# leavesnight/VIEO_SLAM

Hardware: AMD Instinct MI355X
Metric: frontend+localBA frames/sec on EuRoC MH05 stereo-VIO; ATE vs ref (higher is better)
Workload: dtype u8 (extract/match) + f64 (pose optimisation)

## Files before the change

### vieo_slam_amd/csrc/orb_extractor.hip

```cpp
#include <algorithm>
#include <cmath>
#include <type_traits>
#include <vector>

#include "../../include/vieo_orb_pattern_31.h"
#include "common.h"
#include "sincosf_exact.h"
#include "wave_ops.h"

#define QT_DEVICE
#include "quadtree.inl"

#include "orb_internal.h"

namespace vieo {

#ifndef VIEO_RESIZE_ROWS
#define VIEO_RESIZE_ROWS 32
#endif
static const int kResizeRows = VIEO_RESIZE_ROWS;
#ifndef VIEO_QT_GROUPS
#define VIEO_QT_GROUPS {1, 64}
#endif

// ... 156 lines not shown
    const short4 y = yt2[dy];
    const uint8_t* r0 = l1 + (y.x - ry0) * kL1P;
    const uint8_t* r1 = l1 + (y.y - ry0) * kL1P;
    const int b0 = y.z, b1 = y.w;
    unsigned out = 0;
#pragma unroll
    for (int j = 0; j < 4; j++) {
      const int h0 = r0[x0[j]] * a0[j] + r0[x1[j]] * a1[j];
      const int h1 = r1[x0[j]] * a0[j] + r1[x1[j]] * a1[j];
      const int v = (((b0 * (int)(unsigned short)(h0 >> 4)) >> 16) + ((b1 * (int)(unsigned short)(h1 >> 4)) >> 16) + 2) >> 2;
      out |= (unsigned)(v & 0xFF) << (8 * j);
    }
    *(unsigned*)(dst2 + (size_t)dy * D2.pitch + dx4) = out & keep;
  }
}

#ifndef VIEO_XCD_RUN
#define VIEO_XCD_RUN 32
#endif
static const int kXcdRun = VIEO_XCD_RUN;
__device__ __forceinline__ int xcd_grouped(int bid, int G) {
  const int xcd = bid & 7, q = bid >> 3;
  return ((q / G) * 8 + xcd) * G + q % G;
}

__device__ __forceinline__ int min3i(int a, int b, int c) { return min(min(a, b), c); }
__device__ __forceinline__ int max3i(int a, int b, int c) { return max(max(a, b), c); }

__device__ __forceinline__ int fast_strength(const uint8_t* t, int p) {
  const int v = t[0];
  int d[16];
  d[0] = v - t[3 * p];
  d[1] = v - t[3 * p + 1];
  d[2] = v - t[2 * p + 2];
  d[3] = v - t[p + 3];
  d[4] = v - t[3];
  d[5] = v - t[-p + 3];
  d[6] = v - t[-2 * p + 2];
  d[7] = v - t[-3 * p + 1];
  d[8] = v - t[-3 * p];
  d[9] = v - t[-3 * p - 1];
  d[10] = v - t[-2 * p - 2];
  d[11] = v - t[-p - 3];
  d[12] = v - t[-3];
  d[13] = v - t[p - 3];
  d[14] = v - t[2 * p - 2];
  d[15] = v - t[3 * p - 1];
  int lo3[16], hi3[16];
#pragma unroll
  for (int k = 0; k < 16; k++) {
    lo3[k] = min3i(d[k], d[(k + 1) & 15], d[(k + 2) & 15]);
    hi3[k] = max3i(d[k], d[(k + 1) & 15], d[(k + 2) & 15]);
  }
  int A = -256, B = 256;
#pragma unroll
  for (int k = 0; k < 16; k++) {
    A = max(A, min3i(lo3[k], lo3[(k + 3) & 15], lo3[(k + 6) & 15]));
    B = min(B, max3i(hi3[k], hi3[(k + 3) & 15], hi3[(k + 6) & 15]));
  }
  return max(max(A, -B), 0);
}

#ifdef VIEO_FAST_STATS
__device__ unsigned long long g_fast_stats[8];
#define FAST_STAT(i, v) do { if (lane == 0) atomicAdd(&g_fast_stats[i], (unsigned long long)(v)); } while (0)
#else
#define FAST_STAT(i, v) do { } while (0)
#endif

__device__ __forceinline__ bool fast_compass(const uint8_t* t, int p, int th) {
  const int v = t[0], lo = v - th, hi = v + th;
  const int x0 = t[3 * p], x4 = t[3], x8 = t[-3 * p], x12 = t[-3];
  const bool dk = ((x0 < lo) | (x8 < lo)) & ((x4 < lo) | (x12 < lo));
  const bool br = ((x0 > hi) | (x8 > hi)) & ((x4 > hi) | (x12 > hi));
  return dk | br;
}

__device__ __forceinline__ void wave_sync() {
  __builtin_amdgcn_fence(__ATOMIC_RELEASE, "wavefront");
  __builtin_amdgcn_wave_barrier();
  __builtin_amdgcn_fence(__ATOMIC_ACQUIRE, "wavefront");
}

__device__ __forceinline__ void fast_cell(const OrbParams& P, const CellDesc& cd, int b, int c, uint8_t* tile, uint8_t* sc,
                                          unsigned short* cand, int cand_cap, int tpitch, int iniTh, int minTh, int lane,
                                          unsigned* __restrict__ cell_keys, int* __restrict__ cell_counts) {
  const int x0a = cd.x0 & ~3;
  const int vw = cd.cw - 6, vh = cd.ch - 6;
  const int npx = (vw > 0 && vh > 0) ? vw * vh : 0;
  const int sp = vw + 2;
  if (npx > 0)
    for (int idx = lane; idx < ((vh + 2) * sp + 15) / 16; idx += 64) ((uint4*)sc)[idx] = make_uint4(0, 0, 0, 0);
  wave_sync();
  const int xo = cd.x0 - x0a;
  unsigned* out = cell_keys + ((size_t)b * P.ncells + c) * P.cell_cap;
  int base = 0;
  for (int round = 0; round < 2 && base == 0; round++) {
    if (round == 1 && minTh >= iniTh) break;
    const int th = round == 0 ? iniTh : minTh;
    int na = 0, nc = 0;
    bool overflow = false;
    FAST_STAT(round, 1);
    auto pass_b = [&]() {
      int w = nc;
      FAST_STAT(3, (na - nc + 63) / 64);
      FAST_STAT(6, na - nc);
      for (int i0 = nc; i0 < na; i0 += 64) {
        const int i = i0 + lane;
        bool pass = false;
        int p = 0;
        if (i < na) {
          p = cand[i];
          const int y = p >> 6, x = p & 63;
          const int r = fast_strength(tile + (y + 3) * tpitch + (x + 3 + xo), tpitch);
          sc[(y + 1) * sp + x + 1] = (uint8_t)r;
          pass = r > th;
        }
        const unsigned long long m = __ballot(pass);
        if (pass) cand[w + __popcll(m & ((1ull << lane) - 1ull))] = (unsigned short)p;
        w += __popcll(m);
      }
      nc = na = w;
    };
    if (npx > 0) {
      const int s = __builtin_amdgcn_readfirstlane((3 + xo) & 3), kq = (3 + xo) >> 2;
      const int ng = (vw + 3) >> 2, G = ng * vh;
      const int qy = 64 / ng, rx = 64 - qy * ng;
      const unsigned H = 0x80808080u, T = (unsigned)th * 0x01010101u;
      const unsigned Tl = T & ~H;
      auto ltu = [&](unsigned a, unsigned bb) -> unsigned {
        const unsigned d = (a | H) - (bb & ~H);
        return __builtin_amdgcn_bitop3_b32(a, bb, d, 0x4D);
      };
      auto pass_a = [&](auto SC) {
        constexpr int S = decltype(SC)::value;
        int y = lane / ng, lx4 = lane - y * ng;
        int toff = y * tpitch + 4 * lx4;
        const int step_off = qy * tpitch + 4 * rx, wrap_off = tpitch - 4 * ng;
        const uint8_t* base_u = tile + 4 * kq;
        const uint8_t* base_c = base_u + 3 * tpitch;
        const uint8_t* base_d = base_u + 6 * tpitch;
        const unsigned Htail = (unsigned)(0x80808080ull & ((1ull << (8 * (vw - 4 * (ng - 1)))) - 1ull));
        for (int g0 = 0; g0 < G; g0 += 64) {
          if (na + 256 > cand_cap) {
            wave_sync();
            pass_b();
            wave_sync();
            if (na + 256 > cand_cap) {
              overflow = true;
              break;
            }
          }
          unsigned m4 = 0;
          const int x0 = 4 * lx4;
          if (g0 + lane < G) {
            const unsigned* rc = (const unsigned*)(base_c + toff);
            const unsigned* ru = (const unsigned*)(base_u + toff);
            const unsigned* rd = (const unsigned*)(base_d + toff);
            unsigned C, L, R, U, D;
            if constexpr (S == 0) {
              const unsigned wm = rc[-1], w0 = rc[0], w1 = rc[1];
              C = w0, U = ru[0], D = rd[0], L = __builtin_amdgcn_alignbyte(w0, wm, 1), R = __builtin_amdgcn_alignbyte(w1, w0, 3);
            } else if constexpr (S == 1) {
              const unsigned wm = rc[-1], w0 = rc[0], w1 = rc[1];
              C = __builtin_amdgcn_alignbyte(w1, w0, 1), U = __builtin_amdgcn_alignbyte(ru[1], ru[0], 1),
              D = __builtin_amdgcn_alignbyte(rd[1], rd[0], 1), L = __builtin_amdgcn_alignbyte(w0, wm, 2), R = w1;
            } else if constexpr (S == 2) {
              const unsigned wm = rc[-1], w0 = rc[0], w1 = rc[1], w2 = rc[2];
              C = __builtin_amdgcn_alignbyte(w1, w0, 2), U = __builtin_amdgcn_alignbyte(ru[1], ru[0], 2),
              D = __builtin_amdgcn_alignbyte(rd[1], rd[0], 2), L = __builtin_amdgcn_alignbyte(w0, wm, 3),
              R = __builtin_amdgcn_alignbyte(w2, w1, 1);
            } else {
              const unsigned w0 = rc[0], w1 = rc[1], w2 = rc[2];
              C = __builtin_amdgcn_alignbyte(w1, w0, 3), U = __builtin_amdgcn_alignbyte(ru[1], ru[0], 3),
              D = __builtin_amdgcn_alignbyte(rd[1], rd[0], 3), L = w0, R = __builtin_amdgcn_alignbyte(w2, w1, 2);
            }
            const unsigned ge = ~ltu(C, T) & H;
            const unsigned gem = (ge - (ge >> 7)) | ge;
            const unsigned dif = ((C | H) - Tl) ^ ((C ^ ~T) & H);
            const unsigned lo = dif & gem;
            const unsigned suml = (C & ~H) + Tl;
            const unsigned sum = suml ^ ((C ^ T) & H);
            const unsigned cy = __builtin_amdgcn_bitop3_b32(C, T, suml, 0xE8) & H;
            const unsigned hi = sum | ((cy - (cy >> 7)) | cy);
            const unsigned dk = (ltu(U, lo) | ltu(D, lo)) & (ltu(L, lo) | ltu(R, lo));
            const unsigned br = (ltu(hi, U) | ltu(hi, D)) & (ltu(hi, L) | ltu(hi, R));
            const unsigned f = (dk | br) & (lx4 == ng - 1 ? Htail : H);
            m4 = ((f >> 7) * 0x01020408u) >> 24;
          }
          const int cnt = __popc(m4);
          int inc = cnt;
          inc += __builtin_amdgcn_update_dpp(0, inc, 0x111, 0xF, 0xF, true);
          inc += __builtin_amdgcn_update_dpp(0, inc, 0x112, 0xF, 0xF, true);
          inc += __builtin_amdgcn_update_dpp(0, inc, 0x114, 0xF, 0xF, true);
          inc += __builtin_amdgcn_update_dpp(0, inc, 0x118, 0xF, 0xF, true);
          inc += VIEO_DPP(0, inc, VIEO_DPP_ROW_BCAST15, 0xA);
          inc += VIEO_DPP(0, inc, VIEO_DPP_ROW_BCAST31, 0xC);
          int pos = na + inc - cnt;
          const unsigned key = (unsigned)((y << 6) | x0);
#pragma unroll
          for (int j = 0; j < 4; j++)
            if (m4 & (1u << j)) cand[pos++] = (unsigned short)(key + j);
          na += __builtin_amdgcn_readlane(inc, 63);
          lx4 += rx, y += qy, toff += step_off;
          if (lx4 >= ng) lx4 -= ng, y++, toff += wrap_off;
        }
      };
      if (s == 0) pass_a(std::integral_constant<int, 0>());
      else if (s == 1) pass_a(std::integral_constant<int, 1>());
      else if (s == 2) pass_a(std::integral_constant<int, 2>());
      else pass_a(std::integral_constant<int, 3>());
    }
    wave_sync();
    if (!overflow) pass_b();
    else {
      FAST_STAT(2, 1);
      for (int i0 = 0; i0 < npx; i0 += 64) {
        const int i = i0 + lane;
        if (i < npx) {
          const int y = i / vw, x = i - y * vw;
          sc[(y + 1) * sp + x + 1] = (uint8_t)fast_strength(tile + (y + 3) * tpitch + (x + 3 + xo), tpitch);
        }
      }
    }
    wave_sync();
    const int nC = overflow ? npx : nc;
    FAST_STAT(4, (nC + 63) / 64);
    for (int i0 = 0; i0 < nC; i0 += 64) {
      const int i = i0 + lane;
      bool keep = false;
      unsigned key = 0;
      if (i < nC) {
        int x, y;
        if (overflow) {
          y = i / vw, x = i - y * vw;
        } else {
          const int p = cand[i];
          y = p >> 6, x = p & 63;
        }
        const uint8_t* s = sc + (y + 1) * sp + x + 1;
        const int r = s[0];
        if (r > th) {
          const int sv = r - 1;
#define NB(o) ((s[o] > th) ? (int)s[o] - 1 : 0)
          keep = sv > NB(1) && sv > NB(-1) && sv > NB(-sp - 1) && sv > NB(-sp) && sv > NB(-sp + 1) &&
                 sv > NB(sp - 1) && sv > NB(sp) && sv > NB(sp + 1);
#undef NB
          key = (unsigned)(x + 3 + cd.offx) | ((unsigned)(y + 3 + cd.offy) << 12) |
                ((unsigned)sv << 24);
        }
      }
      const unsigned long long m = __ballot(keep);
      if (keep) {
        const int pos = base + __popcll(m & ((1ull << lane) - 1ull));
        if (pos < P.cell_cap) out[pos] = key;
      }
      base += __popcll(m);
    }
    wave_sync();
  }
  FAST_STAT(7, base);
  if (lane == 0) cell_counts[(size_t)b * P.ncells + c] = min(base, P.cell_cap);
}

#ifndef VIEO_FAST_WAVES
#define VIEO_FAST_WAVES 1
#endif
__global__ void __launch_bounds__(64 * VIEO_FAST_WAVES)
k_fast(OrbParams P, ImgSet I, const CellDesc* __restrict__ cells, unsigned* __restrict__ cell_keys,
       int* __restrict__ cell_counts, int iniTh, int minTh, int tpitch, int tile_bytes,
       int score_bytes, int cand_cap, int n_images, int lds_per_wave) {
  extern __shared__ __attribute__((aligned(16))) uint8_t smem_all[];
  const int lane = threadIdx.x & 63;
  const int wave_in_wg = __builtin_amdgcn_readfirstlane((int)(threadIdx.x >> 6));
  uint8_t* smem = smem_all + wave_in_wg * lds_per_wave;
  const int item = xcd_grouped(blockIdx.x, kXcdRun) * VIEO_FAST_WAVES + wave_in_wg;
  if (item >= P.ncells * n_images) return;
  const int b = item / P.ncells, c = item - b * P.ncells;
  const CellDesc cd = cells[c];
  int pitch;
  const uint8_t* src = plane_ptr(P, I, b, cd.level, &pitch);
  uint8_t* tile = smem;
  uint8_t* sc = smem + tile_bytes;
  unsigned short* cand = (unsigned short*)(smem + tile_bytes + score_bytes);
  const int x0a = cd.x0 & ~3;
  const int ndw = ((cd.x0 + cd.cw + 3) >> 2) - (x0a >> 2);
  {
    const int dc = lane & 15, dr = lane >> 4;
    const uint8_t* gbase = src + (size_t)cd.y0 * pitch + x0a;
    const unsigned gstep = 4u * (unsigned)pitch, tstep = 4u * (unsigned)tpitch;
    unsigned goff = (unsigned)dr * (unsigned)pitch + 4u * dc;
    uint8_t* t = tile + dr * tpitch + 4 * dc;
    const int kfull = cd.ch >> 2;
    if (dc < ndw) {
      unsigned v[16];
#pragma unroll
      for (int k = 0; k < 16; k++) {
        if (k < kfull)
          v[k] = *(const unsigned*)(gbase + goff);
        else if (dr + 4 * k < cd.ch)
          v[k] = *(const unsigned*)(gbase + goff);
        goff += gstep;
      }
#pragma unroll
      for (int k = 0; k < 16; k++) {
        if (k < kfull)
          *(unsigned*)t = v[k];
        else if (dr + 4 * k < cd.ch)
          *(unsigned*)t = v[k];
        t += tstep;
      }
      for (int r = dr + 64; r < cd.ch; r += 4, goff += gstep, t += tstep) *(unsigned*)t = *(const unsigned*)(gbase + goff);
    }
    for (int idx = lane; idx < cd.ch * (ndw - 16); idx += 64) {
      const int r = idx / (ndw - 16), dcol = 16 + idx % (ndw - 16);
      *(unsigned*)(tile + r * tpitch + 4 * dcol) =
          *(const unsigned*)(src + (size_t)(cd.y0 + r) * pitch + x0a + 4 * dcol);
    }
  }
  fast_cell(P, cd, b, c, tile, sc, cand, cand_cap, tpitch, iniTh, minTh, lane, cell_keys, cell_counts);
}

__global__ void __launch_bounds__(1024)
k_quadtree(OrbParams P, const unsigned* __restrict__ cell_keys,
           const int* __restrict__ cell_counts, unsigned* __restrict__ keys,
           unsigned short* __restrict__ kslot, unsigned char* __restrict__ kq,
           unsigned* __restrict__ sel, int* __restrict__ sel_count, int ncap_max, int scap_max, int l0) {
  extern __shared__ __attribute__((aligned(16))) uint8_t smem[];
  const int l = l0 + blockIdx.x, b = blockIdx.y;
  const LevelDesc& D = P.lv[l];
  uint8_t* q = smem;
  QtMem m;
  m.scanA = (unsigned long long*)q;
  q += sizeof(unsigned long long) * scap_max;
  m.scanB = (unsigned long long*)q;
  q += sizeof(unsigned long long) * scap_max;
  m.cnt = (int*)q;
  q += 4 * ncap_max;
  m.cc = (int*)q;
  q += 16 * ncap_max;
  m.best = (unsigned*)q;
  q += 4 * ncap_max;
  m.cand_size[0] = (int*)q;
  q += 4 * ncap_max;
  m.cand_size[1] = (int*)q;
  q += 4 * ncap_max;
  m.s = (QtShared*)q;
  q += 64;
  m.x0 = (short*)q;
  q += 2 * ncap_max;
  m.y0 = (short*)q;
  q += 2 * ncap_max;
  m.x1 = (short*)q;
  q += 2 * ncap_max;
  m.y1 = (short*)q;
  q += 2 * ncap_max;
  m.child = (unsigned short*)q;
  q += 8 * ncap_max;
  m.mark = (unsigned short*)q;
  q += 2 * ncap_max;
  m.list[0] = (unsigned short*)q;
  q += 2 * ncap_max;
  m.list[1] = (unsigned short*)q;
  q += 2 * ncap_max;
  m.cand_slot[0] = (unsigned short*)q;
  q += 2 * ncap_max;
  m.cand_slot[1] = (unsigned short*)q;
  q += 2 * ncap_max;
  m.order = (unsigned short*)q;
  q += 2 * ncap_max;
  m.flag = (unsigned char*)q;
  m.ncap = D.ncap;
  m.scap = scap_max;

  const int tid = threadIdx.x;
  const int ncell = D.cell_end - D.cell_begin;
  const int* cnts = cell_counts + (size_t)b * P.ncells + D.cell_begin;
  for (int i = tid; i < ncell; i += blockDim.x) m.scanA[i] = (unsigned long long)cnts[i];
  for (int i = tid; i < D.nIni; i += blockDim.x) m.cnt[i] = 0;
  __syncthreads();
  unsigned long long* inc = qt_scan(m.scanA, m.scanB, ncell);
  if (tid == 0) m.s->K = ncell > 0 ? (int)inc[ncell - 1] : 0;
  __syncthreads();
  const int K = m.s->K;
  unsigned* kk = keys + (size_t)b * P.keys_per_image + D.key_off;
  unsigned short* ks = kslot + (size_t)b * P.keys_per_image + D.key_off;
  unsigned char* kqq = kq + (size_t)b * P.keys_per_image + D.key_off;
  {
    const unsigned* cells0 = cell_keys + ((size_t)b * P.ncells + D.cell_begin) * P.cell_cap;
    const int nth = blockDim.x;
    for (int t0 = tid; t0 < K; t0 += 4 * nth) {
      unsigned key[4];
#pragma unroll
      for (int u = 0; u < 4; u++) {
        const int t = t0 + u * nth;
        key[u] = 0;
        if (t < K) {
          int lo = 0, hi = ncell - 1;
          while (lo < hi) {
            const int mid = (lo + hi) >> 1;
            if ((int)inc[mid] > t)
              hi = mid;
            else
// ... 706 lines not shown
    if (l > 0) {
      std::vector<short> t;
      D.xtab_off = (int)(xtab.size() / 4);
      resize_axis_table(P.lv[l - 1].w, D.w, true, t);
      xtab.insert(xtab.end(), t.begin(), t.end());
      D.ytab_off = (int)(ytab.size() / 4);
      resize_axis_table(P.lv[l - 1].h, D.h, false, t);
      ytab.insert(ytab.end(), t.begin(), t.end());
      const short* xt = xtab.data() + 4 * (size_t)D.xtab_off;
      const short* yt = ytab.data() + 4 * (size_t)D.ytab_off;
      for (int y0 = 0; y0 < D.h; y0 += kResizeRows)
        resize_rows = std::max(resize_rows, yt[4 * (std::min(y0 + kResizeRows, D.h) - 1) + 1] - yt[4 * y0] + 1);
      for (int x0 = 0; x0 < D.w; x0 += 256)
        resize_dw = std::max(resize_dw, ((xt[4 * (std::min(x0 + 256, D.w) - 1) + 1] + 4) >> 2) - (xt[4 * x0] >> 2));
    }
    D.tile_begin = (int)e->tiles.size();
    D.tiles_x = (D.w + kBlurTW - 1) / kBlurTW;
    for (int ty = 0; ty < (D.h + kBlurTH - 1) / kBlurTH; ty++)
      for (int tx = 0; tx < D.tiles_x; tx++) e->tiles.push_back({(short)l, (short)tx, (short)ty, 0});
    D.tile_end = (int)e->tiles.size();
  }
  P.ncells = (int)e->cells.size();
  if (max_cw - 6 > 64 || max_ch - 6 > 1023) {
    set_error("FAST cell wider than 64 pixels (image narrower than one 30-pixel cell?)");
    return VIEO_E_INVALID;
  }
  P.cell_cap = std::max(16, ((max_cw - 6 + 1) / 2) * ((max_ch - 6 + 1) / 2));
  for (int l = 0; l < e->nlevels; l++) {
    LevelDesc& D = P.lv[l];
    D.key_off = key_off;
    D.key_cap = (D.cell_end - D.cell_begin) * P.cell_cap;
    key_off += D.key_cap;
    if (D.key_cap >= (1 << 24)) {
      set_error("too many candidate keys per level");
      return VIEO_E_INVALID;
    }
  }
  P.keys_per_image = key_off;
  P.sel_per_image = sel_off;
  P.kp_cap = sel_off;
  e->ncap_max = ncap_max;
  e->scap_max = std::max(2 * ncap_max, max_ncell);
  e->pyr_img = align_up_sz(pyr_off, 256);
  e->blur_img = align_up_sz(blur_off, 256);
  e->resize_pitch = 4 * resize_dw + 4;
  e->resize_lds = resize_rows * e->resize_pitch;
  {
    bool ok = e->nlevels >= 3;
    int rows2 = 1, dw2 = 1;
    for (int l = 1; ok && l + 1 < e->nlevels; l += 2) {
      const LevelDesc &D1 = P.lv[l], &D2 = P.lv[l + 1];
      const short* xt1 = xtab.data() + 4 * (size_t)D1.xtab_off;
      const short* yt1 = ytab.data() + 4 * (size_t)D1.ytab_off;
      const short* xt2 = xtab.data() + 4 * (size_t)D2.xtab_off;
      const short* yt2 = ytab.data() + 4 * (size_t)D2.ytab_off;
      for (int ex0 = 0; ok && ex0 < D2.w; ex0 += kR2W) {
        const int ex1 = std::min(ex0 + kR2W, D2.w);
        const int rx0 = ex0 == 0 ? 0 : (xt2[4 * ex0] & ~3), rx1 = ex1 == D2.w ? D1.w : std::min(xt2[4 * (ex1 - 1) + 1] + 1, D1.w);
        const int ox1 = ex1 == D2.w ? D1.w : (xt2[4 * ex1] & ~3);
        const int ndw = ((xt1[4 * (rx1 - 1) + 1] + 4) >> 2) - ((xt1[4 * rx0] & ~3) >> 2);
        ok = rx1 - rx0 <= 256 && ox1 <= rx1 && ox1 > rx0 && ndw <= 128;
        dw2 = std::max(dw2, ndw);
      }
      for (int ey0 = 0; ok && ey0 < D2.h; ey0 += kR2H) {
        const int ey1 = std::min(ey0 + kR2H, D2.h);
        const int ry0 = ey0 == 0 ? 0 : yt2[4 * ey0], ry1 = ey1 == D2.h ? D1.h : std::min(yt2[4 * (ey1 - 1) + 1] + 1, D1.h);
        const int oy1 = ey1 == D2.h ? D1.h : yt2[4 * ey1];
        const int nrows = yt1[4 * (ry1 - 1) + 1] - yt1[4 * ry0] + 1;
        ok = ry1 - ry0 <= kR2Rows && oy1 <= ry1 && oy1 > ry0 && nrows <= 48;
        rows2 = std::max(rows2, nrows);
      }
    }
    e->resize2_ok = ok;
    e->resize2_pitch = 4 * dw2 + 4;
    e->resize2_l1_off = (rows2 * e->resize2_pitch + 15) & ~15;
    e->resize2_lds = e->resize2_l1_off + kR2Rows * 260;
  }
  e->tpitch = align_up(max_cw + 3, 4) + 4;
  e->tile_bytes = align_up(e->tpitch * max_ch, 16);
  e->score_bytes = align_up((max_cw - 4) * (max_ch - 4), 16) + 16;
  e->fast_cand_cap = std::max(256, std::min((max_cw - 6) * (max_ch - 6), 512));
  if (const char* cc = getenv("VIEO_FAST_CAND_CAP")) e->fast_cand_cap = std::max(256, atoi(cc));
  e->fast_lds = e->tile_bytes + e->score_bytes + align_up(2 * e->fast_cand_cap, 16) + 16;
  e->qt_lds = 16 * e->scap_max + (4 + 16 + 4 + 4 + 4) * ncap_max + 64 + (2 * 4 + 8 + 2 * 6) * ncap_max +
              ncap_max + 64;
  int rc;
#define ENS(buf, bytes)                 \
  if ((rc = (buf).ensure(bytes)) != VIEO_OK) return rc
  ENS(e->d_pyr, e->pyr_img * B);
  if (!orb_fused()) ENS(e->d_blur, e->blur_img * B);
  ENS(e->d_cells, e->cells.size() * sizeof(CellDesc));
  ENS(e->d_tiles, e->tiles.size() * sizeof(BlurTile));
  ENS(e->d_xtab, std::max<size_t>(xtab.size() * 2, 8));
  ENS(e->d_ytab, std::max<size_t>(ytab.size() * 2, 8));
  ENS(e->d_cell_keys, (size_t)B * P.ncells * P.cell_cap * 4);
  ENS(e->d_cell_counts, (size_t)B * P.ncells * 4);
  ENS(e->d_keys, (size_t)B * P.keys_per_image * 4);
  ENS(e->d_kslot, (size_t)B * P.keys_per_image * 2);
  ENS(e->d_kq, (size_t)B * P.keys_per_image);
  ENS(e->d_sel, (size_t)B * P.sel_per_image * 4);
  ENS(e->d_sel_count, (size_t)B * kMaxLevels * 4);
  ENS(e->d_tmp_kp, (size_t)B * P.kp_cap * sizeof(vieo_keypoint));
  ENS(e->d_tmp_desc, (size_t)B * P.kp_cap * 32);
  ENS(e->d_tmp_counts, (size_t)B * 2 * 4);
  ENS(e->d_krec, (size_t)B * P.kp_cap * 8);
#undef ENS
  VIEO_HIP_CHECK(hipMemcpyAsync(e->d_cells.p, e->cells.data(), e->cells.size() * sizeof(CellDesc),
                                hipMemcpyHostToDevice, e->stream));
  VIEO_HIP_CHECK(hipMemcpyAsync(e->d_tiles.p, e->tiles.data(), e->tiles.size() * sizeof(BlurTile),
                                hipMemcpyHostToDevice, e->stream));
  if (!xtab.empty()) {
    VIEO_HIP_CHECK(hipMemcpyAsync(e->d_xtab.p, xtab.data(), xtab.size() * 2, hipMemcpyHostToDevice,
                                  e->stream));
    VIEO_HIP_CHECK(hipMemcpyAsync(e->d_ytab.p, ytab.data(), ytab.size() * 2, hipMemcpyHostToDevice,
                                  e->stream));
  }
  VIEO_HIP_CHECK(hipStreamSynchronize(e->stream));
  if (e->qt_lds > 64 * 1024)
    VIEO_HIP_CHECK(hipFuncSetAttribute((const void*)k_quadtree,
                                       hipFuncAttributeMaxDynamicSharedMemorySize, e->qt_lds));
  if (e->qt_lds > 160 * 1024) {
    set_error("nfeatures too large for the LDS quadtree (%d bytes)", e->qt_lds);
    return VIEO_E_INVALID;
  }
  e->w = w;
  e->h = h;
  e->B = B;
  return VIEO_OK;
}

static int run_batch(vieo_orb* e, const uint8_t* d_images, int B, int w, int h, int stride,
                     size_t image_pitch, const int* lapping, vieo_keypoint* d_kp, uint8_t* d_desc,
                     int capacity, int32_t* d_counts) {
  int rc;
  if (w != e->w || h != e->h || B > e->B) {
    if ((rc = plan_geometry(e, w, h, std::max(B, (w == e->w && h == e->h) ? e->B : 0))) != VIEO_OK)
      return rc;
  }
  if ((stride & 3) || ((uintptr_t)d_images & 3) || (image_pitch & 3)) {
    set_error("device images need 4-byte aligned base, stride and pitch");
    return VIEO_E_INVALID;
  }
  const OrbParams& P = e->P;
  ImgSet I;
  I.img0 = d_images;
  I.stride0 = stride;
  I.img_pitch = image_pitch;
  I.pyr = e->d_pyr.as<uint8_t>();
  I.pyr_img = e->pyr_img;
  I.blur = e->d_blur.as<uint8_t>();
  I.blur_img = e->blur_img;
  e->last_imgs = I;
  e->last_B = B;
  hipStream_t st = e->stream;
  Timing& T = e->tm;
  int evi = 0;
  hipEvent_t* evs = T.ev[T.steps % kTimingRing];
#define STAMP()                                                  \
  if (T.on) VIEO_HIP_CHECK(hipEventRecord(evs[evi++], st))
  STAMP();
  static const bool resize_pairs = [] {
    const char* v = getenv("VIEO_RESIZE_PAIRS");
    return !(v && atoi(v) == 0);
  }();
  for (int l = 1; l < P.nlevels;) {
    if (resize_pairs && e->resize2_ok && (l & 1) && l + 1 < P.nlevels) {
      const LevelDesc& D2 = P.lv[l + 1];
      dim3 grd((D2.w + kR2W - 1) / kR2W, (D2.h + kR2H - 1) / kR2H, B);
      hipLaunchKernelGGL(k_resize2, grd, dim3(256), e->resize2_lds, st, P, l, I, e->d_xtab.as<short4>(), e->d_ytab.as<short4>(),
                         e->resize2_pitch, e->resize2_l1_off);
      l += 2;
      continue;
    }
    const LevelDesc& D = P.lv[l];
    dim3 grd((D.w + 255) / 256, (D.h + kResizeRows - 1) / kResizeRows, B);
    hipLaunchKernelGGL(k_resize, grd, dim3(256), e->resize_lds, st, P, l, I, e->d_xtab.as<short4>(),
                       e->d_ytab.as<short4>(), e->resize_pitch);
    l++;
  }
  STAMP();
  const auto xcd_grid = [](long long items) {
    return (unsigned)((items + 8 * kXcdRun - 1) / (8 * kXcdRun) * (8 * kXcdRun));
  };
  if ((long long)P.ncells * B > 0x7FFF0000LL || (long long)e->tiles.size() * B > 0x7FFF0000LL) {
    set_error("batch too large for one launch");
    return VIEO_E_CAPACITY;
  }
  hipLaunchKernelGGL(k_fast, dim3(xcd_grid(((long long)P.ncells * B + VIEO_FAST_WAVES - 1) / VIEO_FAST_WAVES)), dim3(64 * VIEO_FAST_WAVES),
                     (size_t)align_up(e->fast_lds, 16) * VIEO_FAST_WAVES, st, P, I,
                     e->d_cells.as<CellDesc>(), e->d_cell_keys.as<unsigned>(), e->d_cell_counts.as<int>(),
                     e->iniTh, e->minTh, e->tpitch, e->tile_bytes, e->score_bytes, e->fast_cand_cap, B,
                     (int)align_up(e->fast_lds, 16));
  STAMP();
  {
    static const int bounds_batch[] = VIEO_QT_GROUPS;
    static const int bounds_one[] = {64};
    const bool batch = B >= 32;
    const int* bounds = batch ? bounds_batch : bounds_one;
    const size_t n_bounds = batch ? sizeof(bounds_batch) / sizeof(bounds_batch[0]) : 1;
    auto qt_caps = [&](int la, int lb, int* ncap, int* scap) {
      int nc = 1, mc = 1;
      for (int l = la; l < lb; l++) nc = std::max(nc, P.lv[l].ncap), mc = std::max(mc, P.lv[l].cell_end - P.lv[l].cell_begin);
      *ncap = nc, *scap = std::max(2 * nc, mc);
    };
    int la = 0;
    static const int qt_env = [] {
      const char* e = getenv("VIEO_QT_THREADS");
      const int v = e ? atoi(e) : 0;
      return v > 0 ? std::min(std::max(v / 64 * 64, 64), 1024) : 0;
    }();
    const int qt_threads = qt_env > 0 ? qt_env : (B <= 16 ? 512 : 256);
    for (size_t gi = 0; gi < n_bounds && la < P.nlevels; gi++) {
      const int lb = std::min(bounds[gi], P.nlevels);
      if (lb <= la) continue;
      int nc, sc;
      qt_caps(la, lb, &nc, &sc);
      const size_t lds = (size_t)16 * sc + (4 + 16 + 4 + 4 + 4) * nc + 64 + (2 * 4 + 8 + 2 * 6) * nc + nc + 64;
      hipLaunchKernelGGL(k_quadtree, dim3(lb - la, B), dim3(qt_threads), lds, st, P,
                         e->d_cell_keys.as<unsigned>(), e->d_cell_counts.as<int>(),
                         e->d_keys.as<unsigned>(), e->d_kslot.as<unsigned short>(),
                         e->d_kq.as<unsigned char>(), e->d_sel.as<unsigned>(), e->d_sel_count.as<int>(), nc, sc, la);
      la = lb;
    }
  }
  STAMP();
  const bool fused = orb_fused();
  if (!fused) {
    int rc_b = e->d_blur.ensure(e->blur_img * (size_t)e->B);
    if (rc_b != VIEO_OK) return rc_b;
    I.blur = e->d_blur.as<uint8_t>(), e->last_imgs = I;
    hipLaunchKernelGGL(k_blur, dim3(xcd_grid((long long)e->tiles.size() * B)), dim3(256), 0, st, P, I,
                       e->d_tiles.as<BlurTile>(), (int)e->tiles.size(), B);
  }
  STAMP();
  const int per_group = fused ? 4 * fused_kpw(B) : 4 * VIEO_DESC_KPW;
  const int ngroups = (std::min(P.kp_cap, capacity) + per_group - 1) / per_group;
  auto describe = [&](unsigned grid, vieo_keypoint* kp, uint8_t* desc, int cap, int ng) {
    if (fused)
      hipLaunchKernelGGL(k_describe_fused, dim3(grid), dim3(256), 0, st, P, I, e->d_krec.as<uint2>(), e->d_pattern.as<int>(), kp, desc,
                         cap, ng, B, fused_kpw(B));
    else
      hipLaunchKernelGGL(k_describe, dim3(grid), dim3(256), 0, st, P, I, e->d_krec.as<uint2>(), e->d_pattern.as<int>(), kp, desc, cap,
                         ng, B);
  };
  if (!lapping) {
    hipLaunchKernelGGL(k_desc_index, dim3((P.kp_cap + 255) / 256, B), dim3(256), 0, st, P, e->d_sel.as<unsigned>(),
                       e->d_sel_count.as<int>(), e->d_krec.as<uint2>(), capacity, d_counts);
    describe((unsigned)ngroups * 8 * ((B + 7) / 8), d_kp, d_desc, capacity, ngroups);
  } else {
    const int ng = (P.kp_cap + per_group - 1) / per_group;
    hipLaunchKernelGGL(k_desc_index, dim3((P.kp_cap + 255) / 256, B), dim3(256), 0, st, P, e->d_sel.as<unsigned>(),
                       e->d_sel_count.as<int>(), e->d_krec.as<uint2>(), P.kp_cap, e->d_tmp_counts.as<int>());
    describe((unsigned)ng * 8 * ((B + 7) / 8), e->d_tmp_kp.as<vieo_keypoint>(), e->d_tmp_desc.as<uint8_t>(), P.kp_cap, ng);
    hipLaunchKernelGGL(k_lapping, dim3(B), dim3(256), 0, st, e->d_tmp_kp.as<vieo_keypoint>(),
                       e->d_tmp_desc.as<uint8_t>(), P.kp_cap, d_kp, d_desc, capacity,
                       e->d_tmp_counts.as<int>(), d_counts, lapping[0], lapping[1]);
  }
  STAMP();
#undef STAMP
  if (T.on) T.steps++;
  VIEO_HIP_CHECK(hipGetLastError());
  return VIEO_OK;
}

}

extern "C" {

int vieo_orb_create(vieo_orb** out, int nfeatures, float scale_factor, int nlevels, int ini_th,
                    int min_th) {
  const char* pe = getenv("VIEO_ORB_PRIORITY");
  return vieo::orb_create_with_priority(out, nfeatures, scale_factor, nlevels, ini_th, min_th, pe && atoi(pe) > 0 ? 1 : 0);
}

}
// ... 384 lines not shown
```

### vieo_slam_amd/csrc/orb_internal.h

```cpp
#pragma once
#include <vector>

#include "common.h"

namespace vieo {

static const int kPatchSize = 31, kHalfPatch = 15, kEdge = 19;
static const int kMaxLevels = 16;
#ifndef VIEO_BLUR_TH
#define VIEO_BLUR_TH 96
#endif
static const int kBlurTW = 64, kBlurTH = VIEO_BLUR_TH;

struct LevelDesc {
  int w, h, pitch, off;
  int boff;
  int cell_begin, cell_end;
  int nfeat;
  int regW, regH, nIni;
  float hX;
  int key_off, key_cap;
  int sel_off, ncap;
  int xtab_off, ytab_off;
  float scale;
  int patch;
  int tile_begin, tile_end, tiles_x;
};

struct OrbParams {
  int nlevels, cell_cap, ncells, keys_per_image, sel_per_image, kp_cap;
  int umax[kHalfPatch + 1];
  LevelDesc lv[kMaxLevels];
};

struct CellDesc {
  short level, x0, y0, cw, ch, offx, offy, pad;
};

struct ImgSet {
  const uint8_t* img0;
  int stride0;
  size_t img_pitch;
  uint8_t* pyr;
  size_t pyr_img;
  uint8_t* blur;
  size_t blur_img;
};

__device__ __forceinline__ const uint8_t* plane_ptr(const OrbParams& P, const ImgSet& I, int b,
                                                    int l, int* pitch) {
  if (l == 0) {
    *pitch = I.stride0;
    return I.img0 + (size_t)b * I.img_pitch;
  }
  *pitch = P.lv[l].pitch;
  return I.pyr + (size_t)b * I.pyr_img + P.lv[l].off;
}

struct BlurTile {
  short level, tx, ty, pad;
};

static const int kTimingRing = 64;
struct Timing {
  bool on = false;
  hipEvent_t ev[kTimingRing][VIEO_ORB_NSTAGES] = {};
  long steps = 0;
};

int orb_create_with_priority(vieo_orb** out, int nfeatures, float scale_factor, int nlevels, int ini_th, int min_th, int priority);

}

struct vieo_orb {
  int nfeatures, nlevels, iniTh, minTh;
  double scaleFactor;
  std::vector<float> scale, inv_scale, sigma2, inv_sigma2;
  std::vector<int> feats;
  int umax[vieo::kHalfPatch + 1];
  hipStream_t stream = nullptr;
  int w = 0, h = 0, B = 0;
  vieo::OrbParams P;
  std::vector<vieo::CellDesc> cells;
  std::vector<vieo::BlurTile> tiles;
  int tpitch = 0, fast_cand_cap = 0, tile_bytes = 0, score_bytes = 0, fast_lds = 0, qt_lds = 0, ncap_max = 0, scap_max = 0;
  int resize_pitch = 0, resize_lds = 0;
  int resize2_pitch = 0, resize2_l1_off = 0, resize2_lds = 0;
  bool resize2_ok = false;
  size_t pyr_img = 0, blur_img = 0;
  vieo::DevBuf d_pyr, d_blur, d_cells, d_tiles, d_xtab, d_ytab, d_cell_keys, d_cell_counts, d_keys,
      d_kslot, d_kq, d_sel, d_sel_count, d_pattern, d_in, d_kp, d_desc, d_counts, d_tmp_kp,
      d_tmp_desc, d_tmp_counts, d_krec;
  int out_cap = 0;
  int last_B = 0;
  vieo::ImgSet last_imgs{};
  vieo::Timing tm;
  vieo::PinnedBuf h_in, h_res, h_io;
  vieo::DevBuf d_io;
  unsigned long long epoch = 0;
  int res_n = -1, res_mono = 0;
  vieo_keypoint res_sample[16];
  vieo::DevBuf d_uright, d_depth, d_sad;
  unsigned long long uright_epoch = ~0ull;
  std::vector<float> uright_host;
  vieo::DevBuf g_start, g_rec, g_ang;
  unsigned long long grid_epoch = ~0ull;
};
```

Measured before the change: 59120.

## Precompute per-cell FAST plans on host and simplify tile staging and NMS

Per-cell FAST parameters (offsets, grid split, tail mask, clear size, key base) are now computed once on the host into a 64-byte CellPlan struct, replacing the CellDesc-plus-OrbParams derivation done in the kernel. The kernel no longer takes the large OrbParams by value. It replaces the integer division with a magic-multiply, uses a switch-specialized unrolled tile load with a single tail row, and rewrites NMS as a branchless max over the eight neighbours. The aim is to cut scalar and integer work and kernel-argument overhead in k_fast, at the cost of more code paths and a host-side precompute that must stay in sync with the device logic.

```diff
diff --git a/vieo_slam_amd/csrc/orb_extractor.hip b/vieo_slam_amd/csrc/orb_extractor.hip
--- a/vieo_slam_amd/csrc/orb_extractor.hip
+++ b/vieo_slam_amd/csrc/orb_extractor.hip
@@ -262,18 +262,14 @@
   __builtin_amdgcn_fence(__ATOMIC_ACQUIRE, "wavefront");
 }
 
-__device__ __forceinline__ void fast_cell(const OrbParams& P, const CellDesc& cd, int b, int c, uint8_t* tile, uint8_t* sc,
-                                          unsigned short* cand, int cand_cap, int tpitch, int iniTh, int minTh, int lane,
-                                          unsigned* __restrict__ cell_keys, int* __restrict__ cell_counts) {
-  const int x0a = cd.x0 & ~3;
-  const int vw = cd.cw - 6, vh = cd.ch - 6;
-  const int npx = (vw > 0 && vh > 0) ? vw * vh : 0;
-  const int sp = vw + 2;
-  if (npx > 0)
-    for (int idx = lane; idx < ((vh + 2) * sp + 15) / 16; idx += 64) ((uint4*)sc)[idx] = make_uint4(0, 0, 0, 0);
+__device__ __forceinline__ void fast_cell(const CellPlan& cp, uint8_t* tile, uint8_t* sc, unsigned short* cand, int cand_cap,
+                                          int tpitch, int iniTh, int minTh, int lane, unsigned* __restrict__ out, int cell_cap,
+                                          int* __restrict__ cell_count) {
+  const int vw = cp.view & 0xFFFF, vh = cp.view >> 16;
+  const int sp = cp.clear >> 16;
+  for (int idx = lane; idx < (cp.clear & 0xFFFF); idx += 64) ((uint4*)sc)[idx] = make_uint4(0, 0, 0, 0);
   wave_sync();
-  const int xo = cd.x0 - x0a;
-  unsigned* out = cell_keys + ((size_t)b * P.ncells + c) * P.cell_cap;
+  const int xo = cp.align & 255;
   int base = 0;
   for (int round = 0; round < 2 && base == 0; round++) {
     if (round == 1 && minTh >= iniTh) break;
@@ -302,10 +298,10 @@
       }
       nc = na = w;
     };
-    if (npx > 0) {
-      const int s = __builtin_amdgcn_readfirstlane((3 + xo) & 3), kq = (3 + xo) >> 2;
-      const int ng = (vw + 3) >> 2, G = ng * vh;
-      const int qy = 64 / ng, rx = 64 - qy * ng;
+    if (cp.G > 0) {
+      const int s = (cp.align >> 8) & 255, kq = (cp.align >> 16) & 255;
+      const int ng = (int)((unsigned)cp.align >> 24), G = cp.G;
+      const int qy = cp.split & 255, rx = (cp.split >> 8) & 255;
       const unsigned H = 0x80808080u, T = (unsigned)th * 0x01010101u;
       const unsigned Tl = T & ~H;
       auto ltu = [&](unsigned a, unsigned bb) -> unsigned {
@@ -314,13 +310,13 @@
       };
       auto pass_a = [&](auto SC) {
         constexpr int S = decltype(SC)::value;
-        int y = lane / ng, lx4 = lane - y * ng;
+        int y = (lane * (int)((unsigned)cp.split >> 16)) >> 12, lx4 = lane - y * ng;
         int toff = y * tpitch + 4 * lx4;
-        const int step_off = qy * tpitch + 4 * rx, wrap_off = tpitch - 4 * ng;
+        const int step_off = cp.step_off, wrap_off = cp.wrap_off;
         const uint8_t* base_u = tile + 4 * kq;
         const uint8_t* base_c = base_u + 3 * tpitch;
         const uint8_t* base_d = base_u + 6 * tpitch;
-        const unsigned Htail = (unsigned)(0x80808080ull & ((1ull << (8 * (vw - 4 * (ng - 1)))) - 1ull));
+        const unsigned Htail = cp.Htail;
         for (int g0 = 0; g0 < G; g0 += 64) {
           if (na + 256 > cand_cap) {
             wave_sync();
@@ -395,110 +391,104 @@
     if (!overflow) pass_b();
     else {
       FAST_STAT(2, 1);
-      for (int i0 = 0; i0 < npx; i0 += 64) {
-        const int i = i0 + lane;
-        if (i < npx) {
-          const int y = i / vw, x = i - y * vw;
-          sc[(y + 1) * sp + x + 1] = (uint8_t)fast_strength(tile + (y + 3) * tpitch + (x + 3 + xo), tpitch);
-        }
-      }
+      for (int y = 0; y < vh; y++)
+        if (lane < vw) sc[(y + 1) * sp + lane + 1] = (uint8_t)fast_strength(tile + (y + 3) * tpitch + (lane + 3 + xo), tpitch);
     }
     wave_sync();
-    const int nC = overflow ? npx : nc;
-    FAST_STAT(4, (nC + 63) / 64);
-    for (int i0 = 0; i0 < nC; i0 += 64) {
-      const int i = i0 + lane;
-      bool keep = false;
-      unsigned key = 0;
-      if (i < nC) {
-        int x, y;
-        if (overflow) {
-          y = i / vw, x = i - y * vw;
-        } else {
-          const int p = cand[i];
-          y = p >> 6, x = p & 63;
-        }
-        const uint8_t* s = sc + (y + 1) * sp + x + 1;
-        const int r = s[0];
-        if (r > th) {
-          const int sv = r - 1;
-#define NB(o) ((s[o] > th) ? (int)s[o] - 1 : 0)
-          keep = sv > NB(1) && sv > NB(-1) && sv > NB(-sp - 1) && sv > NB(-sp) && sv > NB(-sp + 1) &&
-                 sv > NB(sp - 1) && sv > NB(sp) && sv > NB(sp + 1);
-#undef NB
-          key = (unsigned)(x + 3 + cd.offx) | ((unsigned)(y + 3 + cd.offy) << 12) |
-                ((unsigned)sv << 24);
-        }
-      }
+    auto nms = [&](int x, int y, bool valid) {
+      const uint8_t* s = sc + y * sp + x;
+      const int r = s[sp + 1];
+      const int n0 = max3i(s[0], s[1], s[2]), n1 = max3i(s[sp], s[sp + 2], s[2 * sp]);
+      const int nmax = max3i(n0, n1, max((int)s[2 * sp + 1], (int)s[2 * sp + 2]));
+      const int sv = r - 1;
+      const bool keep = valid & (r > th) & (sv > (nmax > th ? nmax - 1 : 0));
+      const unsigned key = (unsigned)cp.kbase + (unsigned)x + ((unsigned)y << 12) + ((unsigned)sv << 24);
       const unsigned long long m = __ballot(keep);
       if (keep) {
         const int pos = base + __popcll(m & ((1ull << lane) - 1ull));
-        if (pos < P.cell_cap) out[pos] = key;
+        if (pos < cell_cap) out[pos] = key;
       }
       base += __popcll(m);
+    };
+    if (!overflow) {
+      FAST_STAT(4, (nc + 63) / 64);
+      for (int i0 = 0; i0 < nc; i0 += 64) {
+        const int i = i0 + lane;
+        const int p = cand[min(i, nc - 1)];
+        nms(p & 63, p >> 6, i < nc);
+      }
+    } else {
+      FAST_STAT(4, vh);
+      const int x = min(lane, vw - 1);
+      for (int y = 0; y < vh; y++) nms(x, y, lane < vw);
     }
     wave_sync();
   }
   FAST_STAT(7, base);
-  if (lane == 0) cell_counts[(size_t)b * P.ncells + c] = min(base, P.cell_cap);
+  if (lane == 0) *cell_count = min(base, cell_cap);
 }
 
 #ifndef VIEO_FAST_WAVES
 #define VIEO_FAST_WAVES 1
 #endif
 __global__ void __launch_bounds__(64 * VIEO_FAST_WAVES)
-k_fast(OrbParams P, ImgSet I, const CellDesc* __restrict__ cells, unsigned* __restrict__ cell_keys,
-       int* __restrict__ cell_counts, int iniTh, int minTh, int tpitch, int tile_bytes,
-       int score_bytes, int cand_cap, int n_images, int lds_per_wave) {
+k_fast(ImgSet I, const CellPlan* __restrict__ cells, unsigned* __restrict__ cell_keys, int* __restrict__ cell_counts,
+       int iniTh, int minTh, int tpitch, int tile_bytes, int score_bytes, int cand_cap, int n_items, int ncells,
+       int cell_cap, unsigned div_mul, int div_shift, int lds_per_wave) {
   extern __shared__ __attribute__((aligned(16))) uint8_t smem_all[];
   const int lane = threadIdx.x & 63;
   const int wave_in_wg = __builtin_amdgcn_readfirstlane((int)(threadIdx.x >> 6));
   uint8_t* smem = smem_all + wave_in_wg * lds_per_wave;
   const int item = xcd_grouped(blockIdx.x, kXcdRun) * VIEO_FAST_WAVES + wave_in_wg;
-  if (item >= P.ncells * n_images) return;
-  const int b = item / P.ncells, c = item - b * P.ncells;
-  const CellDesc cd = cells[c];
-  int pitch;
-  const uint8_t* src = plane_ptr(P, I, b, cd.level, &pitch);
+  if (item >= n_items) return;
+  const int b = div_mul ? (int)(__umulhi((unsigned)item, div_mul) >> div_shift) : item, c = item - b * ncells;
+  const CellPlan cp = cells[c];
+  const bool level0 = cp.pitch == 0;
+  const int pitch = level0 ? I.stride0 : cp.pitch;
+  const uint8_t* gbase = (level0 ? I.img0 + (size_t)b * I.img_pitch : I.pyr + (size_t)b * I.pyr_img) + (size_t)cp.row * pitch + cp.off;
   uint8_t* tile = smem;
   uint8_t* sc = smem + tile_bytes;
   unsigned short* cand = (unsigned short*)(smem + tile_bytes + score_bytes);
-  const int x0a = cd.x0 & ~3;
-  const int ndw = ((cd.x0 + cd.cw + 3) >> 2) - (x0a >> 2);
-  {
-    const int dc = lane & 15, dr = lane >> 4;
-    const uint8_t* gbase = src + (size_t)cd.y0 * pitch + x0a;
-    const unsigned gstep = 4u * (unsigned)pitch, tstep = 4u * (unsigned)tpitch;
-    unsigned goff = (unsigned)dr * (unsigned)pitch + 4u * dc;
-    uint8_t* t = tile + dr * tpitch + 4 * dc;
-    const int kfull = cd.ch >> 2;
-    if (dc < ndw) {
-      unsigned v[16];
-#pragma unroll
-      for (int k = 0; k < 16; k++) {
-        if (k < kfull)
-          v[k] = *(const unsigned*)(gbase + goff);
-        else if (dr + 4 * k < cd.ch)
-          v[k] = *(const unsigned*)(gbase + goff);
-        goff += gstep;
-      }
-#pragma unroll
-      for (int k = 0; k < 16; k++) {
-        if (k < kfull)
-          *(unsigned*)t = v[k];
-        else if (dr + 4 * k < cd.ch)
-          *(unsigned*)t = v[k];
-        t += tstep;
-      }
-      for (int r = dr + 64; r < cd.ch; r += 4, goff += gstep, t += tstep) *(unsigned*)t = *(const unsigned*)(gbase + goff);
-    }
-    for (int idx = lane; idx < cd.ch * (ndw - 16); idx += 64) {
-      const int r = idx / (ndw - 16), dcol = 16 + idx % (ndw - 16);
-      *(unsigned*)(tile + r * tpitch + 4 * dcol) =
-          *(const unsigned*)(src + (size_t)(cd.y0 + r) * pitch + x0a + 4 * dcol);
-    }
-  }
-  fast_cell(P, cd, b, c, tile, sc, cand, cand_cap, tpitch, iniTh, minTh, lane, cell_keys, cell_counts);
+  const int ch = cp.rows & 0xFFFF, ndw = (cp.rows >> 16) & 255;
+  const int dr = lane >> 4;
+  if (!(cp.rows >> 24)) {
+    {
+      const int dc = min(lane & 15, ndw - 1);
+      const unsigned gstep = 4u * (unsigned)pitch, tstep = 4u * (unsigned)tpitch;
+      const unsigned goff0 = (unsigned)dr * (unsigned)pitch + 4u * dc;
+      const unsigned goff_tail = goff0 + (unsigned)(ch - 4) * (unsigned)pitch;
+      uint8_t* const t0 = tile + dr * tpitch + 4 * dc;
+      auto stage = [&](auto NF) {
+        constexpr int N = decltype(NF)::value;
+        unsigned v[N + 1];
+        unsigned goff = goff0;
+#pragma unroll
+        for (int k = 0; k < N; k++, goff += gstep) v[k] = *(const unsigned*)(gbase + goff);
+        v[N] = *(const unsigned*)(gbase + goff_tail);
+        uint8_t* t = t0;
+#pragma unroll
+        for (int k = 0; k < N; k++, t += tstep) *(unsigned*)t = v[k];
+        *(unsigned*)(t0 + cp.tail_toff) = v[N];
+      };
+#define VIEO_FAST_STAGE(n) case n: stage(std::integral_constant<int, n>()); break;
+      switch ((ch - 1) >> 2) {
+        VIEO_FAST_STAGE(0) VIEO_FAST_STAGE(1) VIEO_FAST_STAGE(2) VIEO_FAST_STAGE(3) VIEO_FAST_STAGE(4) VIEO_FAST_STAGE(5)
+        VIEO_FAST_STAGE(6) VIEO_FAST_STAGE(7) VIEO_FAST_STAGE(8) VIEO_FAST_STAGE(9) VIEO_FAST_STAGE(10) VIEO_FAST_STAGE(11)
+        VIEO_FAST_STAGE(12) VIEO_FAST_STAGE(13) VIEO_FAST_STAGE(14) VIEO_FAST_STAGE(15)
+        default: break;
+      }
+#undef VIEO_FAST_STAGE
+    }
+  } else {
+#pragma clang loop unroll(disable)
+    for (int r = dr; r < ch; r += 4) {
+#pragma clang loop vectorize(disable) interleave(disable) unroll(disable)
+      for (int d = lane & 15; d < ndw; d += 16)
+        *(unsigned*)(tile + r * tpitch + 4 * d) = *(const unsigned*)(gbase + (size_t)r * pitch + 4 * d);
+    }
+  }
+  fast_cell(cp, tile, sc, cand, cand_cap, tpitch, iniTh, minTh, lane, cell_keys + (size_t)item * cell_cap, cell_cap,
+            cell_counts + item);
 }
 
 __global__ void __launch_bounds__(1024)
@@ -1371,6 +1361,40 @@
   e->fast_cand_cap = std::max(256, std::min((max_cw - 6) * (max_ch - 6), 512));
   if (const char* cc = getenv("VIEO_FAST_CAND_CAP")) e->fast_cand_cap = std::max(256, atoi(cc));
   e->fast_lds = e->tile_bytes + e->score_bytes + align_up(2 * e->fast_cand_cap, 16) + 16;
+  std::vector<CellPlan> plans(e->cells.size());
+  for (size_t i = 0; i < e->cells.size(); i++) {
+    const CellDesc& c = e->cells[i];
+    const LevelDesc& D = P.lv[c.level];
+    CellPlan& p = plans[i];
+    memset(&p, 0, sizeof(p));
+    const int x0a = c.x0 & ~3, xo = c.x0 - x0a;
+    const int ndw = ((c.x0 + c.cw + 3) >> 2) - (x0a >> 2);
+    if (c.level == 0) p.off = x0a, p.row = c.y0, p.pitch = 0;
+    else p.off = D.off + c.y0 * D.pitch + x0a, p.row = 0, p.pitch = D.pitch;
+    p.rows = c.ch | ndw << 16 | (ndw > 16 || c.ch > 64 || c.ch < 4 ? 1 << 24 : 0);
+    p.tail_toff = (c.ch - 4) * e->tpitch;
+    p.kbase = (3 + c.offx) | (3 + c.offy) << 12;
+    const int vw = c.cw - 6, vh = c.ch - 6;
+    if (vw > 0 && vh > 0) {
+      const int ng = (vw + 3) >> 2, qy = 64 / ng, rx = 64 - qy * ng, m = (4096 + ng - 1) / ng;
+      p.view = vw | vh << 16;
+      p.align = xo | ((3 + xo) & 3) << 8 | ((3 + xo) >> 2) << 16 | ng << 24;
+      p.split = qy | rx << 8 | m << 16;
+      p.G = ng * vh;
+      p.step_off = qy * e->tpitch + 4 * rx;
+      p.wrap_off = e->tpitch - 4 * ng;
+      p.Htail = (unsigned)(0x80808080ull & ((1ull << (8 * (vw - 4 * (ng - 1)))) - 1ull));
+      p.clear = ((vh + 2) * (vw + 2) + 15) / 16 | (vw + 2) << 16;
+    }
+  }
+  if (P.ncells > 1) {
+    int L = 1;
+    while ((1 << L) < P.ncells) L++;
+    e->cell_div_mul = (unsigned)((((unsigned long long)1 << (31 + L)) + P.ncells - 1) / P.ncells);
+    e->cell_div_shift = L - 1;
+  } else {
+    e->cell_div_mul = 0, e->cell_div_shift = 0;
+  }
   e->qt_lds = 16 * e->scap_max + (4 + 16 + 4 + 4 + 4) * ncap_max + 64 + (2 * 4 + 8 + 2 * 6) * ncap_max +
               ncap_max + 64;
   int rc;
@@ -1378,7 +1402,7 @@
   if ((rc = (buf).ensure(bytes)) != VIEO_OK) return rc
   ENS(e->d_pyr, e->pyr_img * B);
   if (!orb_fused()) ENS(e->d_blur, e->blur_img * B);
-  ENS(e->d_cells, e->cells.size() * sizeof(CellDesc));
+  ENS(e->d_cells, plans.size() * sizeof(CellPlan));
   ENS(e->d_tiles, e->tiles.size() * sizeof(BlurTile));
   ENS(e->d_xtab, std::max<size_t>(xtab.size() * 2, 8));
   ENS(e->d_ytab, std::max<size_t>(ytab.size() * 2, 8));
@@ -1394,7 +1418,7 @@
   ENS(e->d_tmp_counts, (size_t)B * 2 * 4);
   ENS(e->d_krec, (size_t)B * P.kp_cap * 8);
 #undef ENS
-  VIEO_HIP_CHECK(hipMemcpyAsync(e->d_cells.p, e->cells.data(), e->cells.size() * sizeof(CellDesc),
+  VIEO_HIP_CHECK(hipMemcpyAsync(e->d_cells.p, plans.data(), plans.size() * sizeof(CellPlan),
                                 hipMemcpyHostToDevice, e->stream));
   VIEO_HIP_CHECK(hipMemcpyAsync(e->d_tiles.p, e->tiles.data(), e->tiles.size() * sizeof(BlurTile),
                                 hipMemcpyHostToDevice, e->stream));
@@ -1476,10 +1500,10 @@
     return VIEO_E_CAPACITY;
   }
   hipLaunchKernelGGL(k_fast, dim3(xcd_grid(((long long)P.ncells * B + VIEO_FAST_WAVES - 1) / VIEO_FAST_WAVES)), dim3(64 * VIEO_FAST_WAVES),
-                     (size_t)align_up(e->fast_lds, 16) * VIEO_FAST_WAVES, st, P, I,
-                     e->d_cells.as<CellDesc>(), e->d_cell_keys.as<unsigned>(), e->d_cell_counts.as<int>(),
-                     e->iniTh, e->minTh, e->tpitch, e->tile_bytes, e->score_bytes, e->fast_cand_cap, B,
-                     (int)align_up(e->fast_lds, 16));
+                     (size_t)align_up(e->fast_lds, 16) * VIEO_FAST_WAVES, st, I,
+                     e->d_cells.as<CellPlan>(), e->d_cell_keys.as<unsigned>(), e->d_cell_counts.as<int>(),
+                     e->iniTh, e->minTh, e->tpitch, e->tile_bytes, e->score_bytes, e->fast_cand_cap, P.ncells * B, P.ncells,
+                     P.cell_cap, e->cell_div_mul, e->cell_div_shift, (int)align_up(e->fast_lds, 16));
   STAMP();
   {
     static const int bounds_batch[] = VIEO_QT_GROUPS;
diff --git a/vieo_slam_amd/csrc/orb_internal.h b/vieo_slam_amd/csrc/orb_internal.h
--- a/vieo_slam_amd/csrc/orb_internal.h
+++ b/vieo_slam_amd/csrc/orb_internal.h
@@ -36,6 +36,24 @@
 struct CellDesc {
   short level, x0, y0, cw, ch, offx, offy, pad;
 };
+
+struct alignas(16) CellPlan {
+  int off;
+  int row;
+  int pitch;
+  int rows;
+  int view;
+  int align;
+  int split;
+  int G;
+  int step_off, wrap_off;
+  unsigned Htail;
+  int clear;
+  int kbase;
+  int tail_toff;
+  int pad0, pad1;
+};
+static_assert(sizeof(CellPlan) == 64, "CellPlan is one 64-byte scalar load");
 
 struct ImgSet {
   const uint8_t* img0;
@@ -83,6 +101,8 @@
   vieo::OrbParams P;
   std::vector<vieo::CellDesc> cells;
   std::vector<vieo::BlurTile> tiles;
+  unsigned cell_div_mul = 0;
+  int cell_div_shift = 0;
   int tpitch = 0, fast_cand_cap = 0, tile_bytes = 0, score_bytes = 0, fast_lds = 0, qt_lds = 0, ncap_max = 0, scap_max = 0;
   int resize_pitch = 0, resize_lds = 0;
   int resize2_pitch = 0, resize2_l1_off = 0, resize2_lds = 0;
```

Measured after the change: 60490, median of 6. 1.02x the previous value.
